# JuliaParallel/DistributedArrays.jl

Hardware: AMD Instinct MI355X
Metric: sum(DArray) GB/s (higher is better)
Workload: dtype f64; 1 GPU; cfg2: sum(drand(Float64, 2^28)) per GPU, 1-D block distribution; per_gpu_elems=268435456, global_elems=268435456

## Files before the change

distributedarrays_jl_amd/_ffi.py:

```python
import ctypes
import os

_HERE = os.path.dirname(os.path.abspath(__file__))
_SO = os.path.join(_HERE, "libdarray_hip.so")

if not os.path.exists(_SO):
    raise ImportError(
        "libdarray_hip.so is missing (%s). Build it first: "
        "`python -c \"import __graft_entry__; __graft_entry__.build()\"` "
        "or `make -C distributedarrays_jl_amd/csrc`. There is no CPU "
        "fallback: the HIP extension IS the compute path." % _SO)

try:
    ctypes.CDLL("/opt/rocm/lib/libamdhip64.so", mode=ctypes.RTLD_GLOBAL)
except OSError:
    pass

lib = ctypes.CDLL(_SO)

u64 = ctypes.c_uint64
i64 = ctypes.c_int64
i32 = ctypes.c_int
f64 = ctypes.c_double
ptr = ctypes.c_void_p
# ... 57 lines not shown
    "da_sendrecv": ([ptr, i32, ptr, i32, u64], i32),
    "da_p2p_stream": ([i32], i32),
    "da_comm_after_compute": ([], i32),
    "da_main_after_comm": ([], i32),
    "da_comm_sync": ([], i32),
    "da_bcast": ([ptr, u64, i32], i32),
    "da_barrier": ([], i32),
    "da_synchronize": ([], i32),
    "da_event_create": ([ctypes.POINTER(ptr)], i32),
    "da_event_record": ([ptr], i32),
    "da_event_elapsed": ([ptr, ptr, ctypes.POINTER(ctypes.c_float)], i32),
    "da_event_destroy": ([ptr], i32),
    "da_errstr": ([i32], ctypes.c_char_p),
    "da_device_props": ([ctypes.c_char_p, i32, ctypes.POINTER(u64)], i32),
    "da_bytes_in_use": ([], u64),
}

_dbg_sigs = {
    "dbg_reduce_dims_variant": ([u64, u64, u64], i32),
    "dbg_gemm_path": ([i64, i64, i64], i32),
}
_scan_dbg_sigs = {
    "dbg_scan_variant": ([u64, u64, u64], i32),
}
DIMS_VARIANTS = ("slices", "threads", "waves", "blocks")
GEMM_PATHS = ("naive", "mfma")
SCAN_VARIANTS = ("cols", "block", "spans")
COPY_FAMILIES = ("runs", "general")
COPY_MAXND = 6

# ... 18 lines not shown
```

distributedarrays_jl_amd/csrc/abi.hip:

```cpp
#include "common.hpp"
#include <stdarg.h>
#include <stdio.h>
#include <stdlib.h>
#include <unistd.h>
#include <errno.h>
#include <time.h>

namespace da {

static State g_state;
State& st() { return g_state; }

char g_errbuf[1024] = "ok";

int set_err(int code, const char* fmt, ...) {
    va_list ap;
    va_start(ap, fmt);
    vsnprintf(g_errbuf, sizeof(g_errbuf), fmt, ap);
    va_end(ap);
    return code;
}

int ensure_scratch(size_t bytes) {
    if (st().scratch_bytes >= bytes) return 0;
// ... 45 lines not shown
int da_init(int device, int rank, int nranks, const char* rccl_uid_path) {
    if (st().inited) return 0;
    if (nranks < 1 || rank < 0 || rank >= nranks)
        return set_err(-2, "da_init: bad rank %d/%d", rank, nranks);
    DA_CHECK_HIP(hipSetDevice(device));
    DA_CHECK_HIP(hipStreamCreateWithFlags(&st().stream, hipStreamNonBlocking));
    DA_CHECK_HIP(hipStreamCreateWithFlags(&st().comm_stream,
                                          hipStreamNonBlocking));
    DA_CHECK_HIP(hipEventCreateWithFlags(&st().ev_main,
                                         hipEventDisableTiming));
    DA_CHECK_HIP(hipEventCreateWithFlags(&st().ev_comm,
                                         hipEventDisableTiming));
    DA_CHECK_HIP(hipMalloc(&st().red_ticket, sizeof(unsigned int)));
    DA_CHECK_HIP(hipMemset(st().red_ticket, 0, sizeof(unsigned int)));
    st().red_base = 0;
    DA_CHECK_HIP(hipHostMalloc(&st().red_host, 16, hipHostMallocDefault));
    memset(st().red_host, 0, 16);
    DA_CHECK_HIP(hipHostGetDevicePointer(&st().red_host_dev,
                                         st().red_host, 0));
    st().device = device;
    st().rank = rank;
    st().nranks = nranks;
    if (nranks > 1) {
        if (!rccl_uid_path)
            return set_err(-2, "da_init: nranks>1 needs a uid path");
        ncclUniqueId uid;
        if (rank == 0) {
            DA_CHECK_NCCL(ncclGetUniqueId(&uid));
            char tmp[1024];
            snprintf(tmp, sizeof(tmp), "%s.tmp", rccl_uid_path);
            FILE* f = fopen(tmp, "wb");
            if (!f) return set_err(-4, "da_init: cannot write %s", tmp);
// ... 381 lines not shown
    return dbg_mfma_probe_impl(DA_F32, A, B, nullptr, out_raw, st().stream);
}

int dbg_reduce_dims_variant(uint64_t inner, uint64_t axis, uint64_t outer) {
    return reduce_dims_variant(inner, axis, outer);
}

int dbg_gemm_path(int64_t m, int64_t n, int64_t k) {
    return gemm_path(m, n, k);
}

int dbg_scan_variant(uint64_t inner, uint64_t axis, uint64_t outer) {
    return scan_variant(inner, axis, outer);
}


int da_group_start(void) {
    DA_REQUIRE_INIT();
    DA_CHECK_NCCL(ncclGroupStart());
    return 0;
}

int da_group_end(void) {
    DA_REQUIRE_INIT();
    DA_CHECK_NCCL(ncclGroupEnd());
    return 0;
}

static hipStream_t p2p_stream() {
    return st().p2p_comm ? st().comm_stream : st().stream;
// ... 131 lines not shown
```

distributedarrays_jl_amd/csrc/common.hpp:

```cpp
#pragma once
#include <hip/hip_runtime.h>
#include <rccl/rccl.h>
#include <stdint.h>
#include <stdio.h>
#include <string.h>
#include <mutex>
#include <unordered_map>

#include "darray_hip.h"

namespace da {

struct State {
    bool inited = false;
    int device = 0;
    int rank = 0;
    int nranks = 1;
    hipStream_t stream = nullptr;
    hipStream_t comm_stream = nullptr;
    bool p2p_comm = false;
    hipEvent_t ev_main = nullptr, ev_comm = nullptr;
    ncclComm_t comm = nullptr;
    void* scratch = nullptr;
    size_t scratch_bytes = 0;
    void* partials = nullptr;
    size_t partials_bytes = 0;
    unsigned int* red_ticket = nullptr;
    unsigned int red_base = 0;
    void* red_host = nullptr;
    void* red_host_dev = nullptr;
    std::mutex mem_mtx;
    std::unordered_map<void*, uint64_t> allocs;
    uint64_t bytes_in_use = 0;
    std::unordered_map<uint64_t, std::vector<void*>> pool;
    uint64_t pool_bytes = 0;
};

State& st();

extern char g_errbuf[1024];
int set_err(int code, const char* fmt, ...);

#define DA_CHECK_HIP(expr) do {                                          \
    hipError_t _e = (expr);                                              \
    if (_e != hipSuccess)                                                \
// ... 17 lines not shown
    switch (dtype) {
        case DA_F64: return 8;
        case DA_F32: return 4;
        case DA_I64: return 8;
    }
    return 0;
}

int ensure_scratch(size_t bytes);
int ensure_partials(size_t bytes);

constexpr int RMAXB = 8192;
int reduce_grid(uint64_t want);
bool reduce_fused_on();
int reduce_stage2_launch(int redop, int g, int dtype, hipStream_t s);
int reduce_result(void* out_host, size_t bytes, hipStream_t s);

template <typename L>
inline int fanin_launch(int g, L launch) {
    DA_CHECK_HIP(launch(st().red_base));
    st().red_base += (unsigned int)g;
    return 0;
}

int launch_fill(void* chunk, double v, uint64_t n, int dtype, hipStream_t s);
int launch_rand(void* chunk, uint64_t n, int dtype, uint64_t seed, int kind,
                uint64_t offset, hipStream_t s);
int launch_map(int opcode, void* dst, const void* src, uint64_t n, int dtype,
               hipStream_t s);
int launch_map2(int opcode, void* dst, const void* a, const void* b,
                uint64_t n, int dtype, hipStream_t s);
int launch_bcast_fma(void* d, const void* a, const void* b, double c,
                     uint64_t n, int dtype, hipStream_t s);
int launch_map2_scalar(int opcode, void* dst, const void* src, double c,
                       int rev, uint64_t n, int dtype, hipStream_t s);
int launch_expr(const int32_t* prog, int plen, void* dst,
                const uint64_t* dst_dims, int nd,
// ... 80 lines not shown
```

distributedarrays_jl_amd/csrc/embedded_src.hpp:

```cpp
#pragma once
static const char embedded_mapops_hpp[] = R"EMBED(// mapops.hpp — the unary/binary scalar functor tables shared by the
// map/map2 kernels (kernels_elementwise.hip) and the fused-broadcast
// expression interpreter (kernels_expr.hip).  ONE source of truth for
// numerics: da_expr of a single-op program is bit-identical to da_map.
//
// Semantics follow the reference's scalar-math list
// (/root/reference/test/darray.jl:775-800) with Julia conventions
// (sign/round/sinc/cosc/mod noted inline); compiled -ffp-contract=off.
#pragma once
#include "darray_hip.h"
#include "fastmath.hpp"

namespace da {

// -------------------------------------------------------------------- map
// Unary functors.  Julia-compatible semantics noted where non-obvious.
template <typename T> struct MathF;
template <> struct MathF<double> {
    static __device__ double sin_(double x) { return sin(x); }
    static __device__ double cos_(double x) { return cos(x); }
    static __device__ double tan_(double x) { return tan(x); }
    static __device__ double exp_(double x) { return exp(x); }
    static __device__ double log_(double x) { return log(x); }
    static __device__ double sqrt_(double x) { return sqrt(x); }
// ... 382 lines not shown
// ticket - base == g - 1 in unsigned arithmetic; that holds across
// wrap-around, any sequence of grid sizes, and interleaved dtypes /
// reduce / count / expression-reduce calls.
template <typename A>
__device__ __forceinline__ void publish_partial(A* p, A v) {
    if constexpr (sizeof(A) == 8)
        __hip_atomic_store((unsigned long long*)p,
                           __builtin_bit_cast(unsigned long long, v),
                           __ATOMIC_RELAXED, __HIP_MEMORY_SCOPE_AGENT);
    else
        __hip_atomic_store((unsigned int*)p,
                           __builtin_bit_cast(unsigned int, v),
                           __ATOMIC_RELAXED, __HIP_MEMORY_SCOPE_AGENT);
}

// `acc`: the block's partial (valid in thread 0).  `sh`: RTPB/64 + 1
// shared elements — block_reduce_in's scratch plus the "I am last"
// flag, kept in ONE __shared__ object.  Reusing sh[0..3] for the final
// fold is safe: wave 0 read them before it wrote the flag, and every
// other wave writes them again only after the barriers below.
template <typename A>
__device__ __forceinline__ void fanin_finish(int redop, A acc, A* partials,
                                             unsigned int* ticket,
                                             unsigned int base, A* out,
                                             A* sh) {
    if (threadIdx.x == 0) {
        publish_partial(partials + blockIdx.x, acc);
        __asm__ volatile("s_waitcnt vmcnt(0)" ::: "memory");
        unsigned int t = __hip_atomic_fetch_add(
            ticket, 1u, __ATOMIC_RELAXED, __HIP_MEMORY_SCOPE_AGENT);
        sh[RTPB / 64] = (t - base == gridDim.x - 1) ? (A)1 : (A)0;
    }
    __syncthreads();
    if (sh[RTPB / 64] == (A)0) return;
    // guide order: the fence, that lane's vmcnt wait, the barrier
    if (threadIdx.x == 0) {
        __builtin_amdgcn_fence(__ATOMIC_ACQUIRE, "agent");
        __asm__ volatile("s_waitcnt vmcnt(0)" ::: "memory");
    }
    __syncthreads();
    A facc = RedIdent<A>::get(redop);
    for (unsigned int j = threadIdx.x; j < gridDim.x; j += RTPB)
        facc = red_comb(redop, facc, partials[j]);
    facc = block_reduce_in(redop, facc, sh);
    if (threadIdx.x == 0) out[0] = facc;
}

} // namespace da
)EMBED";
static const char embedded_darray_hip_h[] = R"EMBED(/* darray_hip.h — C ABI of libdarray_hip.so: the MI355X-native local-compute
 * path for DistributedArrays.jl-style distributed arrays.
 *
 * This is the drop-in boundary of SURVEY.md §8(b): each entry point replaces
 * one worker-side local operation of the reference (citations below are
 * file:line into /root/reference).  The reference touches localparts only
 * through the init-constructor / localpart / fan-out seam
 * (src/darray.jl:76-118, :330-337; src/broadcast.jl:80; src/mapreduce.jl:31;
 * src/linalg.jl:224), so a Julia caller binds these with plain `ccall`
 * (see INTEGRATION.md) and keeps every other line of the reference.
 *
// ... 170 lines not shown
 * hipRTC (cached per process; DA_EXPR_JIT=0 forces the interpreter).
 * state: 1 ready, 2 active, -1 hipRTC failed (interpreter fallback). */
int da_expr_jit_state(void);
const char* da_expr_jit_errstr(void);
/* Fused mapreduce over a program: op-folds (da_expr_reduce) or counts the
 * nonzero terms of (da_expr_count; exact, NaN counts) the program's values
 * over a local chunk of n elements WITHOUT materialising them — one
 * launch, one read per operand element, result in *out (host; the dtype's
 * own scalar / an int64_t).  Program arguments as da_expr; dims is the
 * local chunk shape reduced over; src_strides == NULL means every operand
 * is dense over it (f64/f32/i64, any n), else the strided variant
 * (f64/f32, nd <= 4, n < 2^32).  n == 0 gives the fold identity / 0.
 * Fold-order contract: *out has EXACTLY the bits of da_expr into a dense
 * temporary followed by da_reduce(DA_REDF_IDENTITY, redop, tmp, n) /
 * da_count(DA_REDF_NONZERO, tmp, n) in the same process (DA_RV4 does not
 * apply; DA_RED_FUSED=0 and DA_EXPR_JIT=0 are honoured, same bits). */
int da_expr_reduce(const int32_t* prog, int prog_len,
                   const uint64_t* dims, int nd,
                   void* const* srcs, const uint64_t* src_strides, int nsrcs,
                   const double* consts, int nconsts, uint64_t n, int dtype,
                   int redop, void* out);
int da_expr_count(const int32_t* prog, int prog_len,
                  const uint64_t* dims, int nd,
                  void* const* srcs, const uint64_t* src_strides, int nsrcs,
                  const double* consts, int nconsts, uint64_t n, int dtype,
                  int64_t* out);
int da_map2_scalar(int opcode, void* dst, const void* src, double c,
                   int reverse, uint64_t n, int dtype);      /* D .+ 1 etc (scalar broadcast arg, broadcast.jl:124-133) */
int da_axpby(void* y, const void* x, double alpha, double beta,
             uint64_t n, int dtype);                         /* y = alpha*x + beta*y: axpy! linalg.jl:24-34 */
int da_add(void* dest, const void* src, double scale,
           uint64_t n, int dtype);                           /* add!, linalg.jl:62-76 */
int da_scale(void* a, double s, uint64_t n, int dtype);      /* rmul!, linalg.jl:54-59 */
/* dtype conversion (DArray{T2}(D) family); float->i64 rounds half-even */
int da_cast(void* dst, int dst_dtype, const void* src, int src_dtype,
            uint64_t n);

/* ---- reductions -------------------------------------------------------*/
/* Local (per-chunk) mapreduce stage: LDS + wavefront-shuffle tree.
 * Result written to *out as the dtype's own scalar type (f64/f32/i64) —
 * the per-worker mapreduce(f, op, localpart(d)) of mapreduce.jl:31.
 * n == 0 returns the fold identity. */
int da_reduce(int mapop, int redop, const void* src, uint64_t n, int dtype,
              void* out);
/* Exact predicate count (count(f, A), mapreduce.jl:115-122): mapop must be
 * a predicate (DA_REDF_ISNAN / ISFINITE / NONZERO).  The 0/1 values are
 * accumulated in a 64-bit integer on the device whatever the source dtype,
 * so *out is exact for every n (a float accumulator rounds above 2^24).
 * Fold across ranks with da_allreduce(out, 1, DA_I64, DA_RED_ADD). */
int da_count(int mapop, const void* src, uint64_t n, int dtype,
             int64_t* out);
/* Per-chunk dims-reduction (src/mapreduce.jl:42-94, mapreducedim_within):
 * chunk viewed column-major as (inner, axis, outer); dst gets
 * inner*outer elements reduced over axis (identity when axis==0). */
int da_reduce_dims(int mapop, int redop, const void* src, uint64_t inner,
                   uint64_t axis, uint64_t outer, int dtype, void* dst);
/* Inclusive scan (Base.accumulate / cumsum / cumprod) of a local chunk viewed
 * column-major as (inner, axis, outer), along `axis`:
 *   dst[i + inner*(k + axis*o)] =
 *       [carry[i + inner*o] (op)] src[i,0,o] (op) src[i,1,o] (op) .. (op) src[i,k,o]
 * redop is a da_redop (ADD, MUL, MIN, MAX; NaN-propagating min/max and
 * wrap-around i64 exactly as da_reduce), dtype f64/f32/i64, accumulation in
 * the dtype itself; the bracketing of a float sum or product is unspecified
 * (a tree over tiles and spans), like the reductions'.  carry is a device
// ... 89 lines not shown
enum da_dims_variant { DA_DIMS_SLICES = 0, DA_DIMS_THREADS, DA_DIMS_WAVES,
                       DA_DIMS_BLOCKS };
enum da_gemm_path_id { DA_GEMM_NAIVE = 0, DA_GEMM_MFMA = 1 };
/* cols: inner > 1, one thread per line; block: inner == 1, one workgroup
 * per line (>= 512 lines, or lines of at most one 2048-element tile);
 * spans: inner == 1, fewer and longer lines, cut into spans, two launches */
enum da_scan_variant { DA_SCAN_COLS = 0, DA_SCAN_BLOCK, DA_SCAN_SPANS };
/* kernel family da_reduce_dims picks for a (inner, axis, outer) view */
int dbg_reduce_dims_variant(uint64_t inner, uint64_t axis, uint64_t outer);
/* MFMA or naive kernel for da_gemm_f64/f32 at (m, n, k), k > 0, alpha != 0 */
int dbg_gemm_path(int64_t m, int64_t n, int64_t k);
/* kernel family da_scan picks for a (inner, axis, outer) view (spelled
 * `extern int`: tests/test_abi.py pins the set of plain `int dbg_*`
 * declarations to the two selectors above) */
extern int dbg_scan_variant(uint64_t inner, uint64_t axis, uint64_t outer);

/* ---- introspection / errors ------------------------------------------ */
const char* da_errstr(int code);
int da_device_props(char* name, int name_len, uint64_t* hbm_bytes);
uint64_t da_bytes_in_use(void);   /* leak check hook (test/runtests.jl:28-37 analog) */

#ifdef __cplusplus
}
#endif
#endif /* DARRAY_HIP_H */
)EMBED";
```

distributedarrays_jl_amd/csrc/expr_jit.hip:

```cpp
#include "common.hpp"
#include "embedded_src.hpp"
#include <hip/hiprtc.h>
#include <stdlib.h>
#include <string>
#include <unordered_map>
#include <vector>

namespace da {

static_assert(DA_EXPR_MAXARGS == 6 && DA_EXPR_MAXCONSTS == 6 &&
              DA_EXPR_MAXND == 4,
              "JARGS_DECL literal must be kept in sync");
struct JArgs {
    void* dst;
    const void* srcs[DA_EXPR_MAXARGS];
    double consts[DA_EXPR_MAXCONSTS];
    unsigned long long n;
    unsigned int dims[DA_EXPR_MAXND];
    unsigned int str[DA_EXPR_MAXARGS][DA_EXPR_MAXND];
};

namespace {

struct JitEntry {
// ... 183 lines not shown
            "}\n", tname, tname, nd, nd, nsrcs > 0 ? nsrcs : 1,
            nsrcs > 0 ? nsrcs : 1, nd);
        s += buf;
    }
    return s;
}

const char* JRARGS_DECL =
    "struct JRArgs {\n"
    "  JArgs a;\n"
    "  void* partials;\n"
    "  unsigned int* ticket;\n"
    "  void* out;\n"
    "  unsigned int base;\n"
    "  int fused;\n"
    "};\n";

std::string gen_reduce_source(const int32_t* prog, int plen, int dtype,
                              int nd, int nsrcs, bool strided, int redop) {
    const bool count = redop == DA_EXPR_COUNT;
    const char* tname = dtype == DA_F64 ? "double"
                        : dtype == DA_F32 ? "float" : "long long";
    const char* aname = (count || dtype == DA_I64) ? "int64_t" : tname;
    const int rop = count ? (int)DA_RED_ADD : redop;
    std::string s =
        "#ifndef M_PI\n#define M_PI 3.14159265358979323846\n#endif\n"
        "#include \"mapops.hpp\"\n#include \"reduce_core.hpp\"\n";
    s += JARGS_DECL;
    s += JRARGS_DECL;
    s += gen_eval(prog, plen, tname, dtype == DA_I64, strided);
// ... 36 lines not shown
        "  unsigned long long st = (unsigned long long)gridDim.x * "
        "da::RTPB;\n"
        "  %s acc = da::RedIdent<%s>::get(%d);\n"
        "  unsigned long long nv = a.n / 2;\n"
        "  for (unsigned long long j = i; j < nv; j += st) {\n"
        "    %s r0 = term(a, 2 * j);\n"
        "    %s r1 = term(a, 2 * j + 1);\n"
        "    acc = ABSORB(acc, r0);\n"
        "    acc = ABSORB(acc, r1);\n"
        "  }\n"
        "  for (unsigned long long j = 2 * nv + i; j < a.n; j += st)\n"
        "    acc = ABSORB(acc, term(a, j));\n"
        "  acc = da::block_reduce_in(%d, acc, sh);\n"
        "  if (r.fused)\n"
        "    da::fanin_finish(%d, acc, (%s*)r.partials, r.ticket, r.base, "
        "(%s*)r.out, sh);\n"
        "  else if (threadIdx.x == 0)\n"
        "    ((%s*)r.partials)[blockIdx.x] = acc;\n"
        "}\n",
        count ? "count" : "reduce", aname, aname, aname, rop, tname, tname,
        rop, rop, aname, aname, aname);
    s += buf;
    return s;
}

int jit_compile(const std::string& src, std::vector<char>* code) {
    const char* hdr_names[] = {"stdint.h", "darray_hip.h", "mapops.hpp",
                               "fastmath.hpp", "reduce_core.hpp"};
    const char* stdint_stub =
        "#pragma once\n"
        "typedef __INT8_TYPE__ int8_t;\ntypedef __UINT8_TYPE__ uint8_t;\n"
// ... 113 lines not shown
    uint64_t b = (work + 255) / 256;
    if (b > 8192) b = 8192;
    if (b == 0) b = 1;
    DA_CHECK_HIP(hipModuleLaunchKernel(fn, (unsigned)b, 1, 1, 256, 1, 1,
                                       0, s, nullptr, cfg));
    return 0;
}

struct JRArgs {
    JArgs a;
    void* partials;
    unsigned int* ticket;
    void* out;
    unsigned int base;
    int fused;
};

int launch_expr_reduce_jit(const int32_t* prog, int plen,
                           const uint64_t* dims, int nd, void* const* srcs,
                           const uint64_t* src_strides, int nsrcs,
                           const double* consts, int nconsts, uint64_t n,
                           int dtype, int redop, int g, bool fused,
                           hipStream_t s) {
    const char* e = getenv("DA_EXPR_JIT");
    if (e && e[0] == '0') return 1;
    if (g_jit_state < 0) return 1;
    bool strided = src_strides != nullptr;
    std::string src = gen_reduce_source(prog, plen, dtype, nd, nsrcs,
                                        strided, redop);
    hipFunction_t fn;
// ... 6 lines not shown
    JRArgs r;
    memset(&r, 0, sizeof(r));
    for (int i = 0; i < nsrcs; ++i) r.a.srcs[i] = srcs[i];
    for (int i = 0; i < nconsts; ++i) r.a.consts[i] = consts[i];
    r.a.n = n;
    if (strided) {
        for (int d = 0; d < nd; ++d) r.a.dims[d] = (unsigned)dims[d];
        for (int k = 0; k < nsrcs; ++k)
            for (int d = 0; d < nd; ++d)
                r.a.str[k][d] = (unsigned)src_strides[(size_t)k * nd + d];
    }
    r.partials = st().partials;
    r.ticket = st().red_ticket;
    r.out = st().red_host_dev;
    r.fused = fused ? 1 : 0;
    auto launch = [&](unsigned int base) {
        r.base = base;
        size_t rsz = sizeof(r);
        void* cfg[] = {HIP_LAUNCH_PARAM_BUFFER_POINTER, &r,
                       HIP_LAUNCH_PARAM_BUFFER_SIZE, &rsz,
                       HIP_LAUNCH_PARAM_END};
        return hipModuleLaunchKernel(fn, (unsigned)g, 1, 1, 256, 1, 1, 0, s,
                                     nullptr, cfg);
    };
    if (fused) return fanin_launch(g, launch);
    DA_CHECK_HIP(launch(0u));
    return 0;
}

int expr_jit_state() { return g_jit_state; }
const char* expr_jit_err() { return g_jit_err; }

}

extern "C" int dbg_expr_jit_compile(const int32_t* prog, int plen,
                                    int dtype, int nd, int nsrcs,
                                    int strided, char* src_out,
                                    int src_len) {
    using namespace da;
    std::string src = gen_source(prog, plen, dtype, nd, nsrcs,
                                 strided != 0, 1);
// ... 28 lines not shown
```

distributedarrays_jl_amd/csrc/kernels_expr.hip:

```cpp
#include "common.hpp"
#include "mapops.hpp"
#include "reduce_core.hpp"
#include <math.h>

namespace da {

namespace {
constexpr int TPB = 256;
constexpr int MAXBLOCKS = 8192;

static inline int nblocks(uint64_t work) {
    uint64_t b = (work + TPB - 1) / TPB;
    if (b > (uint64_t)MAXBLOCKS) b = MAXBLOCKS;
    if (b == 0) b = 1;
    return (int)b;
}
}

struct ExprProg {
    int32_t ins[DA_EXPR_MAXLEN];
    int len;
    const void* srcs[DA_EXPR_MAXARGS];
    double consts[DA_EXPR_MAXCONSTS];
};
// ... 245 lines not shown
                                                 uint64_t i) {
        return expr_eval_i64(p, i);
    }
};

template <bool COUNT, typename A, typename T>
__device__ __forceinline__ A expr_absorb(int redop, A acc, T x) {
    if constexpr (COUNT) return acc + (x != (T)0 ? 1 : 0);
    else return red_comb(redop, acc, x);
}

template <typename T, typename A, bool COUNT, bool STRIDED>
__global__ void expr_reduce_kernel(ExprProg p, ExprStrides s, uint64_t n,
                                   int redop, A* partials,
                                   unsigned int* ticket, unsigned int base,
                                   int fused, A* out) {
    __shared__ A sh[RTPB / 64 + 1];
    auto term = [&](uint64_t i) -> T {
        if constexpr (STRIDED) return expr_strided_eval<T>(p, s, i);
        else return ExprTerm<T>::at(p, i);
    };
    if (COUNT) redop = DA_RED_ADD;
    uint64_t i = (uint64_t)blockIdx.x * RTPB + threadIdx.x;
    uint64_t stride = (uint64_t)gridDim.x * RTPB;
    A acc = RedIdent<A>::get(redop);
    uint64_t nv = n / 2;
    for (uint64_t j = i; j < nv; j += stride) {
        T r0 = term(2 * j);
        T r1 = term(2 * j + 1);
        acc = expr_absorb<COUNT>(redop, acc, r0);
        acc = expr_absorb<COUNT>(redop, acc, r1);
    }
    for (uint64_t j = 2 * nv + i; j < n; j += stride)
        acc = expr_absorb<COUNT>(redop, acc, term(j));
    acc = block_reduce_in(redop, acc, sh);
    if (fused)
        fanin_finish(redop, acc, partials, ticket, base, out, sh);
    else if (threadIdx.x == 0)
        partials[blockIdx.x] = acc;
}

namespace {
struct ExprRedArgs {
    ExprProg P;
    ExprStrides S;
    uint64_t n;
    int redop, g;
    bool fused;
    hipStream_t s;
};

template <typename T, typename A, bool COUNT, bool STRIDED>
int expr_reduce_interp(const ExprRedArgs& a) {
    A* parts = (A*)st().partials;
    A* out = (A*)st().red_host_dev;
    auto launch = [&](unsigned int base) {
        hipLaunchKernelGGL((expr_reduce_kernel<T, A, COUNT, STRIDED>),
                           dim3(a.g), dim3(RTPB), 0, a.s, a.P, a.S, a.n,
                           a.redop, parts, st().red_ticket, base,
                           a.fused ? 1 : 0, out);
        return hipGetLastError();
    };
    if (a.fused) return fanin_launch(a.g, launch);
    DA_CHECK_HIP(launch(0u));
    return 0;
}

template <typename T, bool STRIDED>
int expr_reduce_interp_t(const ExprRedArgs& a, bool count) {
    return count ? expr_reduce_interp<T, int64_t, true, STRIDED>(a)
                 : expr_reduce_interp<T, T, false, STRIDED>(a);
}
}

int launch_expr_reduce(const int32_t* prog, int plen, const uint64_t* dims,
                       int nd, void* const* srcs,
                       const uint64_t* src_strides, int nsrcs,
                       const double* consts, int nconsts, uint64_t n,
                       int dtype, int redop, void* out_host, hipStream_t s) {
// ... 62 lines not shown
            rc = expr_reduce_interp_t<int64_t, false>(a, count);
        else if (dtype == DA_F64)
            rc = strided ? expr_reduce_interp_t<double, true>(a, count)
                         : expr_reduce_interp_t<double, false>(a, count);
        else
            rc = strided ? expr_reduce_interp_t<float, true>(a, count)
                         : expr_reduce_interp_t<float, false>(a, count);
        if (rc) return rc;
    }
    if (!fused) {
        rc = reduce_stage2_launch(count ? (int)DA_RED_ADD : redop, g,
                                  count ? (int)DA_I64 : dtype, s);
        if (rc) return rc;
    }
    return reduce_result(out_host, count ? sizeof(int64_t)
                                         : dtype_size(dtype), s);
}

}
```

distributedarrays_jl_amd/csrc/kernels_reduce.hip:

```cpp
#include "common.hpp"
#include "reduce_core.hpp"
#include <stdlib.h>

namespace da {

int reduce_grid(uint64_t want) {
    static int cap = -1;
    if (cap < 0) {
        const char* e = getenv("DA_RBLOCKS");
        cap = e ? atoi(e) : 2048;
        if (cap < 1 || cap > RMAXB) cap = 2048;
    }
    if (want < 1) want = 1;
    return (int)(want > (uint64_t)cap ? (uint64_t)cap : want);
}

static inline bool reduce_v4() {
    static int v = -1;
    if (v < 0) {
        const char* e = getenv("DA_RV4");
        v = e ? atoi(e) : 0;
    }
    return v == 1;
}
// ... 25 lines not shown
template <typename T>
__device__ __forceinline__ T block_reduce(int redop, T v) {
    __shared__ T lds[RTPB / 64];
    return block_reduce_in(redop, v, lds);
}

template <int W, typename T, typename A, typename F>
__device__ __forceinline__ A grid_accumulate(const T* __restrict__ src,
                                             uint64_t n, A acc, F fold) {
    uint64_t i = (uint64_t)blockIdx.x * RTPB + threadIdx.x;
    uint64_t stride = (uint64_t)gridDim.x * RTPB;
    using V = T __attribute__((ext_vector_type(W)));
    uint64_t nv = n / W;
    const V* sv = reinterpret_cast<const V*>(src);
    for (uint64_t j = i; j < nv; j += stride) {
        V v = sv[j];
#pragma unroll
        for (int k = 0; k < W; ++k) acc = fold(acc, (T)v[k]);
    }
    for (uint64_t j = W * nv + i; j < n; j += stride)
        acc = fold(acc, src[j]);
    return acc;
}

template <typename T, int MOP = -1, int ROP = -1>
__global__ void reduce_stage1(int mapop, int redop, const T* __restrict__ src,
                              uint64_t n, T* __restrict__ partials) {
    if (MOP >= 0) mapop = MOP;
    if (ROP >= 0) redop = ROP;
    T acc = grid_accumulate<2>(src, n, RedIdent<T>::get(redop),
        [=](T a, T x) { return red_comb(redop, a, mapf<T>(mapop, x)); });
// ... 4 lines not shown
template <typename T, int MOP = -1, int ROP = -1>
__global__ void reduce_stage1_v4(int mapop, int redop,
                                 const T* __restrict__ src, uint64_t n,
                                 T* __restrict__ partials) {
    if (MOP >= 0) mapop = MOP;
    if (ROP >= 0) redop = ROP;
    T acc = grid_accumulate<4>(src, n, RedIdent<T>::get(redop),
        [=](T a, T x) { return red_comb(redop, a, mapf<T>(mapop, x)); });
    acc = block_reduce(redop, acc);
    if (threadIdx.x == 0) partials[blockIdx.x] = acc;
}

template <typename T, int MOP = -1, int ROP = -1>
__global__ void reduce_fused(int mapop, int redop, const T* __restrict__ src,
                             uint64_t n, T* partials, unsigned int* ticket,
                             unsigned int base, T* out) {
    if (MOP >= 0) mapop = MOP;
    if (ROP >= 0) redop = ROP;
    __shared__ T sh[RTPB / 64 + 1];
    T acc = grid_accumulate<2>(src, n, RedIdent<T>::get(redop),
        [=](T a, T x) { return red_comb(redop, a, mapf<T>(mapop, x)); });
    acc = block_reduce_in(redop, acc, sh);
    fanin_finish(redop, acc, partials, ticket, base, out, sh);
}

template <typename T>
__global__ void reduce_stage2(int redop, const T* __restrict__ partials,
                              int np, T* __restrict__ out) {
    T acc = RedIdent<T>::get(redop);
    for (int j = threadIdx.x; j < np; j += blockDim.x)
        acc = red_comb(redop, acc, partials[j]);
    acc = block_reduce(redop, acc);
    if (threadIdx.x == 0) out[0] = acc;
}

bool reduce_fused_on() {
    static int v = -1;
    if (v < 0) {
// ... 3 lines not shown
    return v == 1;
}

template <typename T> struct FlatArgs {
    bool fused;
    int grid, mapop, redop;
    const T* src;
    uint64_t n;
    T *parts, *out;
    hipStream_t s;
};

template <typename T, int MOP, int ROP>
static int launch_flat(const FlatArgs<T>& a) {
    if (a.fused)
        return fanin_launch(a.grid, [&](unsigned int base) {
            hipLaunchKernelGGL((reduce_fused<T, MOP, ROP>), dim3(a.grid),
                               dim3(RTPB), 0, a.s, a.mapop, a.redop, a.src,
                               a.n, a.parts, st().red_ticket, base, a.out);
            return hipGetLastError();
        });
    hipLaunchKernelGGL((reduce_stage1<T, MOP, ROP>), dim3(a.grid),
                       dim3(RTPB), 0, a.s, a.mapop, a.redop, a.src, a.n,
                       a.parts);
    DA_CHECK_HIP(hipGetLastError());
    return 0;
}

template <typename T>
static int do_reduce(int mapop, int redop, const T* src, uint64_t n,
                     void* out_host, hipStream_t s) {
    if (n == 0) {
        *(T*)out_host = RedIdent<T>::get(redop);
        return 0;
// ... 15 lines not shown
        rc = launch_flat<T, DA_REDF_ABS2, DA_RED_ADD>(a);
    else if (mapop == DA_REDF_ABS && redop == DA_RED_ADD)
        rc = launch_flat<T, DA_REDF_ABS, DA_RED_ADD>(a);
    else if (mapop == DA_REDF_IDENTITY && redop == DA_RED_MAX)
        rc = launch_flat<T, DA_REDF_IDENTITY, DA_RED_MAX>(a);
    else if (mapop == DA_REDF_IDENTITY && redop == DA_RED_MIN)
        rc = launch_flat<T, DA_REDF_IDENTITY, DA_RED_MIN>(a);
    else
        rc = launch_flat<T, -1, -1>(a);
    if (rc) return rc;
    if (!a.fused) {
        hipLaunchKernelGGL(reduce_stage2<T>, dim3(1), dim3(RTPB), 0, s,
                           redop, a.parts, g, a.out);
        DA_CHECK_HIP(hipGetLastError());
    }
    return reduce_result(out_host, sizeof(T), s);
}

template <typename T>
__device__ __forceinline__ int64_t predf(int mapop, T x) {
    switch (mapop) {
    case DA_REDF_ISNAN: return x != x ? 1 : 0;
    case DA_REDF_ISFINITE: return isfinite((double)x) ? 1 : 0;
    }
    return x != (T)0 ? 1 : 0;
}
template <>
__device__ __forceinline__ int64_t predf<int64_t>(int mapop, int64_t x) {
    return mapf(mapop, x);
}

template <typename T>
__global__ void count_stage1(int mapop, const T* __restrict__ src,
                             uint64_t n, int64_t* __restrict__ partials) {
    int64_t acc = grid_accumulate<2>(src, n, (int64_t)0,
        [=](int64_t a, T x) { return a + predf<T>(mapop, x); });
    acc = block_reduce(DA_RED_ADD, acc);
    if (threadIdx.x == 0) partials[blockIdx.x] = acc;
}

template <typename T>
__global__ void count_fused(int mapop, const T* __restrict__ src, uint64_t n,
                            int64_t* partials, unsigned int* ticket,
                            unsigned int base, int64_t* out) {
    __shared__ int64_t sh[RTPB / 64 + 1];
    int64_t acc = grid_accumulate<2>(src, n, (int64_t)0,
        [=](int64_t a, T x) { return a + predf<T>(mapop, x); });
    acc = block_reduce_in((int)DA_RED_ADD, acc, sh);
    fanin_finish((int)DA_RED_ADD, acc, partials, ticket, base, out, sh);
}

template <typename T>
static int do_count(int mapop, const T* src, uint64_t n, int64_t* out_host,
                    hipStream_t s) {
    int g = reduce_grid((n / 2 + RTPB - 1) / RTPB);
    int rc = ensure_partials(RMAXB * sizeof(double));
    if (rc) return rc;
    int64_t* parts = (int64_t*)st().partials;
    int64_t* out = (int64_t*)st().red_host_dev;
    if (reduce_fused_on()) {
        rc = fanin_launch(g, [&](unsigned int base) {
            hipLaunchKernelGGL(count_fused<T>, dim3(g), dim3(RTPB), 0, s,
                               mapop, src, n, parts, st().red_ticket, base,
                               out);
            return hipGetLastError();
        });
        if (rc) return rc;
    } else {
        hipLaunchKernelGGL(count_stage1<T>, dim3(g), dim3(RTPB), 0, s,
                           mapop, src, n, parts);
        DA_CHECK_HIP(hipGetLastError());
        hipLaunchKernelGGL(reduce_stage2<int64_t>, dim3(1), dim3(RTPB), 0, s,
                           (int)DA_RED_ADD, parts, g, out);
        DA_CHECK_HIP(hipGetLastError());
    }
    return reduce_result(out_host, sizeof(int64_t), s);
}

int launch_count(int mapop, const void* src, uint64_t n, int dtype,
                 int64_t* out_host, hipStream_t s) {
    if (mapop < DA_REDF_ISNAN || mapop > DA_REDF_NONZERO)
        return set_err(-3, "da_count: mapop %d is not a predicate", mapop);
    if (!out_host) return set_err(-3, "da_count: null out");
    if (dtype != DA_F64 && dtype != DA_F32 && dtype != DA_I64)
        return set_err(-3, "da_count: bad dtype %d", dtype);
    if (n == 0) { *out_host = 0; return 0; }
    switch (dtype) {
    case DA_F64: return do_count<double>(mapop, (const double*)src, n,
                                         out_host, s);
    case DA_F32: return do_count<float>(mapop, (const float*)src, n,
                                        out_host, s);
// ... 223 lines not shown
        break;
    case DA_F32:
        hipLaunchKernelGGL(reduce_stage2<float>, dim3(1), dim3(RTPB), 0, s,
                           redop, (const float*)st().partials, g,
                           (float*)st().red_host_dev);
        break;
    default:
        hipLaunchKernelGGL(reduce_stage2<int64_t>, dim3(1), dim3(RTPB), 0, s,
                           redop, (const int64_t*)st().partials, g,
                           (int64_t*)st().red_host_dev);
    }
    DA_CHECK_HIP(hipGetLastError());
    return 0;
}

int reduce_result(void* out_host, size_t bytes, hipStream_t s) {
    DA_CHECK_HIP(hipStreamSynchronize(s));
    memcpy(out_host, st().red_host, bytes);
    return 0;
}

}
```

distributedarrays_jl_amd/csrc/reduce_core.hpp:

```cpp
#pragma once
#include "darray_hip.h"

namespace da {

constexpr int RTPB = 256;

template <typename T> struct RedIdent {
    static __device__ __host__ T get(int redop) {
        switch (redop) {
        case DA_RED_ADD: return (T)0;
        case DA_RED_MUL: return (T)1;
        case DA_RED_MIN: return (T)__builtin_inff();
        case DA_RED_MAX: return (T)(-__builtin_inff());
        }
        return (T)0;
    }
};
template <> struct RedIdent<int64_t> {
    static __device__ __host__ int64_t get(int redop) {
        switch (redop) {
        case DA_RED_ADD: return 0;
        case DA_RED_MUL: return 1;
        case DA_RED_MIN: return __INT64_MAX__;
        case DA_RED_MAX: return -__INT64_MAX__ - 1;
// ... 44 lines not shown
}

template <typename A>
__device__ __forceinline__ void publish_partial(A* p, A v) {
    if constexpr (sizeof(A) == 8)
        __hip_atomic_store((unsigned long long*)p,
                           __builtin_bit_cast(unsigned long long, v),
                           __ATOMIC_RELAXED, __HIP_MEMORY_SCOPE_AGENT);
    else
        __hip_atomic_store((unsigned int*)p,
                           __builtin_bit_cast(unsigned int, v),
                           __ATOMIC_RELAXED, __HIP_MEMORY_SCOPE_AGENT);
}

template <typename A>
__device__ __forceinline__ void fanin_finish(int redop, A acc, A* partials,
                                             unsigned int* ticket,
                                             unsigned int base, A* out,
                                             A* sh) {
    if (threadIdx.x == 0) {
        publish_partial(partials + blockIdx.x, acc);
        __asm__ volatile("s_waitcnt vmcnt(0)" ::: "memory");
        unsigned int t = __hip_atomic_fetch_add(
            ticket, 1u, __ATOMIC_RELAXED, __HIP_MEMORY_SCOPE_AGENT);
        sh[RTPB / 64] = (t - base == gridDim.x - 1) ? (A)1 : (A)0;
    }
    __syncthreads();
    if (sh[RTPB / 64] == (A)0) return;
    if (threadIdx.x == 0) {
        __builtin_amdgcn_fence(__ATOMIC_ACQUIRE, "agent");
        __asm__ volatile("s_waitcnt vmcnt(0)" ::: "memory");
    }
    __syncthreads();
    A facc = RedIdent<A>::get(redop);
    for (unsigned int j = threadIdx.x; j < gridDim.x; j += RTPB)
        facc = red_comb(redop, facc, partials[j]);
    facc = block_reduce_in(redop, facc, sh);
    if (threadIdx.x == 0) out[0] = facc;
}

}
```

include/darray_hip.h:

```cpp
#ifndef DARRAY_HIP_H
#define DARRAY_HIP_H

#include <stdint.h>

#ifdef __cplusplus
extern "C" {
#endif

enum da_dtype { DA_F64 = 0, DA_F32 = 1, DA_I64 = 2 };

enum da_mapop {
    DA_OP_IDENTITY = 0, DA_OP_NEG, DA_OP_ABS, DA_OP_ABS2, DA_OP_INV,
    DA_OP_SQRT, DA_OP_CBRT, DA_OP_EXP, DA_OP_EXP2, DA_OP_EXP10,
    DA_OP_EXPM1, DA_OP_LOG, DA_OP_LOG2, DA_OP_LOG10, DA_OP_LOG1P,
    DA_OP_SIN, DA_OP_COS, DA_OP_TAN, DA_OP_ASIN, DA_OP_ACOS, DA_OP_ATAN,
    DA_OP_SINH, DA_OP_COSH, DA_OP_TANH, DA_OP_ASINH, DA_OP_ACOSH,
    DA_OP_ATANH, DA_OP_SINPI, DA_OP_COSPI, DA_OP_FLOOR, DA_OP_CEIL,
    DA_OP_ROUND, DA_OP_TRUNC, DA_OP_SIGN, DA_OP_DEG2RAD, DA_OP_RAD2DEG,
    DA_OP_SEC, DA_OP_CSC, DA_OP_COT,
    DA_OP_ERF, DA_OP_ERFC, DA_OP_ERFINV, DA_OP_ERFCINV, DA_OP_ERFCX,
    DA_OP_GAMMA, DA_OP_LGAMMA, DA_OP_SINC, DA_OP_COSC,
    DA_OP_SIND, DA_OP_COSD, DA_OP_TAND, DA_OP_ASIND, DA_OP_ACOSD,
    DA_OP_ATAND, DA_OP_ACOT, DA_OP_ACOTD, DA_OP_ASEC, DA_OP_ACSC,
    DA_OP_ASECH, DA_OP_ACSCH, DA_OP_ACOTH,
// ... 132 lines not shown
int da_barrier(void);

int da_synchronize(void);
int da_event_create(void** ev);
int da_event_record(void* ev);
int da_event_elapsed(void* ev_start, void* ev_stop, float* ms);
int da_event_destroy(void* ev);

enum da_dims_variant { DA_DIMS_SLICES = 0, DA_DIMS_THREADS, DA_DIMS_WAVES,
                       DA_DIMS_BLOCKS };
enum da_gemm_path_id { DA_GEMM_NAIVE = 0, DA_GEMM_MFMA = 1 };
enum da_scan_variant { DA_SCAN_COLS = 0, DA_SCAN_BLOCK, DA_SCAN_SPANS };
int dbg_reduce_dims_variant(uint64_t inner, uint64_t axis, uint64_t outer);
int dbg_gemm_path(int64_t m, int64_t n, int64_t k);
extern int dbg_scan_variant(uint64_t inner, uint64_t axis, uint64_t outer);

const char* da_errstr(int code);
int da_device_props(char* name, int name_len, uint64_t* hbm_bytes);
uint64_t da_bytes_in_use(void);

#ifdef __cplusplus
}
#endif
#endif
```

Before: 6139 GB/s.

## Poll a pinned host result slot instead of synchronising the stream after reductions

The fused single-launch reduce kernels now publish {value, sequence} into a coherent mapped pinned host slot with a system-scope release store. The host spins on that sequence word for up to DA_RED_SPIN_US microseconds before falling back to hipStreamSynchronize, which removes the stream-sync latency from each scalar reduce. The grid-accumulate loop also switches to nontemporal loads of the source. In exchange the host burns CPU while spinning, the stream is no longer guaranteed drained on return, and the slot becomes fine-grained coherent memory.

Measured after the change: 6829 GB/s, median of 6. 1.11x the previous value.

```diff
diff --git a/distributedarrays_jl_amd/_ffi.py b/distributedarrays_jl_amd/_ffi.py
--- a/distributedarrays_jl_amd/_ffi.py
+++ b/distributedarrays_jl_amd/_ffi.py
@@ -95,6 +95,7 @@
     "da_errstr": ([i32], ctypes.c_char_p),
     "da_device_props": ([ctypes.c_char_p, i32, ctypes.POINTER(u64)], i32),
     "da_bytes_in_use": ([], u64),
+    "da_dbg_reduce_waits": ([ctypes.POINTER(u64), ctypes.POINTER(u64)], i32),
 }
 
 _dbg_sigs = {
diff --git a/distributedarrays_jl_amd/csrc/abi.hip b/distributedarrays_jl_amd/csrc/abi.hip
--- a/distributedarrays_jl_amd/csrc/abi.hip
+++ b/distributedarrays_jl_amd/csrc/abi.hip
@@ -83,8 +83,11 @@
     DA_CHECK_HIP(hipMalloc(&st().red_ticket, sizeof(unsigned int)));
     DA_CHECK_HIP(hipMemset(st().red_ticket, 0, sizeof(unsigned int)));
     st().red_base = 0;
-    DA_CHECK_HIP(hipHostMalloc(&st().red_host, 16, hipHostMallocDefault));
+    DA_CHECK_HIP(hipHostMalloc(&st().red_host, 16,
+                               hipHostMallocCoherent | hipHostMallocMapped));
     memset(st().red_host, 0, 16);
+    st().red_seq = 0;
+    reduce_waits_reset();
     DA_CHECK_HIP(hipHostGetDevicePointer(&st().red_host_dev,
                                          st().red_host, 0));
     st().device = device;
@@ -496,6 +499,11 @@
     return scan_variant(inner, axis, outer);
 }
 
+int da_dbg_reduce_waits(uint64_t* polled, uint64_t* synced) {
+    reduce_waits(polled, synced);
+    return 0;
+}
+
 
 int da_group_start(void) {
     DA_REQUIRE_INIT();
diff --git a/distributedarrays_jl_amd/csrc/common.hpp b/distributedarrays_jl_amd/csrc/common.hpp
--- a/distributedarrays_jl_amd/csrc/common.hpp
+++ b/distributedarrays_jl_amd/csrc/common.hpp
@@ -29,6 +29,7 @@
     unsigned int red_base = 0;
     void* red_host = nullptr;
     void* red_host_dev = nullptr;
+    uint64_t red_seq = 0;
     std::mutex mem_mtx;
     std::unordered_map<void*, uint64_t> allocs;
     uint64_t bytes_in_use = 0;
@@ -76,13 +77,28 @@
 int reduce_grid(uint64_t want);
 bool reduce_fused_on();
 int reduce_stage2_launch(int redop, int g, int dtype, hipStream_t s);
-int reduce_result(void* out_host, size_t bytes, hipStream_t s);
+int reduce_result(void* out_host, size_t bytes, hipStream_t s, uint64_t seq);
+void reduce_waits(uint64_t* polled, uint64_t* synced);
+void reduce_waits_reset();
 
 template <typename L>
 inline int fanin_launch(int g, L launch) {
     DA_CHECK_HIP(launch(st().red_base));
     st().red_base += (unsigned int)g;
     return 0;
+}
+
+template <typename L>
+inline int fanin_launch_seq(int g, L launch) {
+    const uint64_t seq = st().red_seq + 1;
+    int rc = fanin_launch(g, [&](unsigned int base) {
+        return launch(base, (unsigned long long)seq);
+    });
+    if (rc == 0) st().red_seq = seq;
+    return rc;
+}
+inline uint64_t published_seq(bool fused) {
+    return fused ? st().red_seq : 0;
 }
 
 int launch_fill(void* chunk, double v, uint64_t n, int dtype, hipStream_t s);
diff --git a/distributedarrays_jl_amd/csrc/embedded_src.hpp b/distributedarrays_jl_amd/csrc/embedded_src.hpp
--- a/distributedarrays_jl_amd/csrc/embedded_src.hpp
+++ b/distributedarrays_jl_amd/csrc/embedded_src.hpp
@@ -420,6 +420,31 @@
                            __ATOMIC_RELAXED, __HIP_MEMORY_SCOPE_AGENT);
 }
 
+// The result hand-off to the host.  `out` is the device address of the
+// 16-byte pinned host slot { 8-byte value, 64-bit sequence } (RedSlot,
+// reduce_wait.hpp).  One lane, once per launch: a system-scope store of
+// the value, then a system-scope RELEASE store of this launch's `seq`
+// into out + 8, so a host whose acquire load of the sequence word
+// returns `seq` reads this launch's value.  The release stays a release:
+// the guide's fence-free write-through form (§6 Guideline 16 R1) is
+// stated for agent-scope hand-offs inside a launch, not for host-visible
+// memory at system scope.  Two stores, never one 16-byte one: nothing
+// promises that arrives untorn.
+template <typename A>
+__device__ __forceinline__ void publish_result(A* out, A v,
+                                               unsigned long long seq) {
+    if constexpr (sizeof(A) == 8)
+        __hip_atomic_store((unsigned long long*)out,
+                           __builtin_bit_cast(unsigned long long, v),
+                           __ATOMIC_RELAXED, __HIP_MEMORY_SCOPE_SYSTEM);
+    else
+        __hip_atomic_store((unsigned int*)out,
+                           __builtin_bit_cast(unsigned int, v),
+                           __ATOMIC_RELAXED, __HIP_MEMORY_SCOPE_SYSTEM);
+    __hip_atomic_store((unsigned long long*)((char*)out + 8), seq,
+                       __ATOMIC_RELEASE, __HIP_MEMORY_SCOPE_SYSTEM);
+}
+
 // `acc`: the block's partial (valid in thread 0).  `sh`: RTPB/64 + 1
 // shared elements — block_reduce_in's scratch plus the "I am last"
 // flag, kept in ONE __shared__ object.  Reusing sh[0..3] for the final
@@ -429,6 +454,7 @@
 __device__ __forceinline__ void fanin_finish(int redop, A acc, A* partials,
                                              unsigned int* ticket,
                                              unsigned int base, A* out,
+                                             unsigned long long seq,
                                              A* sh) {
     if (threadIdx.x == 0) {
         publish_partial(partials + blockIdx.x, acc);
@@ -449,7 +475,7 @@
     for (unsigned int j = threadIdx.x; j < gridDim.x; j += RTPB)
         facc = red_comb(redop, facc, partials[j]);
     facc = block_reduce_in(redop, facc, sh);
-    if (threadIdx.x == 0) out[0] = facc;
+    if (threadIdx.x == 0) publish_result(out, facc, seq);
 }
 
 } // namespace da
@@ -650,7 +676,9 @@
  * Fold-order contract: *out has EXACTLY the bits of da_expr into a dense
  * temporary followed by da_reduce(DA_REDF_IDENTITY, redop, tmp, n) /
  * da_count(DA_REDF_NONZERO, tmp, n) in the same process (DA_RV4 does not
- * apply; DA_RED_FUSED=0 and DA_EXPR_JIT=0 are honoured, same bits). */
+ * apply; DA_RED_FUSED=0 and DA_EXPR_JIT=0 are honoured, same bits).
+ * Like da_reduce, neither call drains the stream (stream contract under
+ * "reductions" below). */
 int da_expr_reduce(const int32_t* prog, int prog_len,
                    const uint64_t* dims, int nd,
                    void* const* srcs, const uint64_t* src_strides, int nsrcs,
@@ -673,17 +701,31 @@
             uint64_t n);
 
 /* ---- reductions -------------------------------------------------------*/
+/* Stream contract of the scalar results (da_reduce, da_count,
+ * da_expr_reduce, da_expr_count): the call returns once *out holds the
+ * result, and by then the reducing kernel has finished READING its
+ * sources.  It does NOT promise that the rank's stream has drained: the
+ * single-launch kernel publishes {value, sequence} into a pinned host slot
+ * and the host watches that slot for up to DA_RED_SPIN_US microseconds
+ * (default 2000) instead of synchronising the stream.  Work queued before
+ * the reduce has completed (one stream, in order); the runtime may not yet
+ * know.  A caller that needs the stream drained (to read other device
+ * results through its own channel, say) calls da_synchronize.  The stream
+ * is synchronised as before when the budget runs out (a kernel fault comes
+ * back as the HIP error then), with DA_RED_SPIN_US=0, and on the
+ * two-kernel path (DA_RED_FUSED=0, DA_RV4=1). */
 /* Local (per-chunk) mapreduce stage: LDS + wavefront-shuffle tree.
  * Result written to *out as the dtype's own scalar type (f64/f32/i64) —
  * the per-worker mapreduce(f, op, localpart(d)) of mapreduce.jl:31.
- * n == 0 returns the fold identity. */
+ * n == 0 returns the fold identity.  Does not drain the stream (above). */
 int da_reduce(int mapop, int redop, const void* src, uint64_t n, int dtype,
               void* out);
 /* Exact predicate count (count(f, A), mapreduce.jl:115-122): mapop must be
  * a predicate (DA_REDF_ISNAN / ISFINITE / NONZERO).  The 0/1 values are
  * accumulated in a 64-bit integer on the device whatever the source dtype,
  * so *out is exact for every n (a float accumulator rounds above 2^24).
- * Fold across ranks with da_allreduce(out, 1, DA_I64, DA_RED_ADD). */
+ * Fold across ranks with da_allreduce(out, 1, DA_I64, DA_RED_ADD).
+ * Does not drain the stream (stream contract above). */
 int da_count(int mapop, const void* src, uint64_t n, int dtype,
              int64_t* out);
 /* Per-chunk dims-reduction (src/mapreduce.jl:42-94, mapreducedim_within):
@@ -803,6 +845,10 @@
  * `extern int`: tests/test_abi.py pins the set of plain `int dbg_*`
  * declarations to the two selectors above) */
 extern int dbg_scan_variant(uint64_t inner, uint64_t axis, uint64_t outer);
+/* how many scalar results (da_reduce, da_count, da_expr_reduce,
+ * da_expr_count) were taken from the poll of the pinned slot and how many
+ * from the stream-sync fallback since da_init; either pointer may be NULL */
+int da_dbg_reduce_waits(uint64_t* polled, uint64_t* synced);
 
 /* ---- introspection / errors ------------------------------------------ */
 const char* da_errstr(int code);
diff --git a/distributedarrays_jl_amd/csrc/expr_jit.hip b/distributedarrays_jl_amd/csrc/expr_jit.hip
--- a/distributedarrays_jl_amd/csrc/expr_jit.hip
+++ b/distributedarrays_jl_amd/csrc/expr_jit.hip
@@ -221,6 +221,7 @@
     "  void* out;\n"
     "  unsigned int base;\n"
     "  int fused;\n"
+    "  unsigned long long seq;\n"
     "};\n";
 
 std::string gen_reduce_source(const int32_t* prog, int plen, int dtype,
@@ -287,7 +288,7 @@
         "  acc = da::block_reduce_in(%d, acc, sh);\n"
         "  if (r.fused)\n"
         "    da::fanin_finish(%d, acc, (%s*)r.partials, r.ticket, r.base, "
-        "(%s*)r.out, sh);\n"
+        "(%s*)r.out, r.seq, sh);\n"
         "  else if (threadIdx.x == 0)\n"
         "    ((%s*)r.partials)[blockIdx.x] = acc;\n"
         "}\n",
@@ -431,6 +432,7 @@
     void* out;
     unsigned int base;
     int fused;
+    unsigned long long seq;
 };
 
 int launch_expr_reduce_jit(const int32_t* prog, int plen,
@@ -467,8 +469,9 @@
     r.ticket = st().red_ticket;
     r.out = st().red_host_dev;
     r.fused = fused ? 1 : 0;
-    auto launch = [&](unsigned int base) {
+    auto launch = [&](unsigned int base, unsigned long long seq) {
         r.base = base;
+        r.seq = seq;
         size_t rsz = sizeof(r);
         void* cfg[] = {HIP_LAUNCH_PARAM_BUFFER_POINTER, &r,
                        HIP_LAUNCH_PARAM_BUFFER_SIZE, &rsz,
@@ -476,8 +479,8 @@
         return hipModuleLaunchKernel(fn, (unsigned)g, 1, 1, 256, 1, 1, 0, s,
                                      nullptr, cfg);
     };
-    if (fused) return fanin_launch(g, launch);
-    DA_CHECK_HIP(launch(0u));
+    if (fused) return fanin_launch_seq(g, launch);
+    DA_CHECK_HIP(launch(0u, 0ull));
     return 0;
 }
 
diff --git a/distributedarrays_jl_amd/csrc/kernels_expr.hip b/distributedarrays_jl_amd/csrc/kernels_expr.hip
--- a/distributedarrays_jl_amd/csrc/kernels_expr.hip
+++ b/distributedarrays_jl_amd/csrc/kernels_expr.hip
@@ -283,7 +283,8 @@
 __global__ void expr_reduce_kernel(ExprProg p, ExprStrides s, uint64_t n,
                                    int redop, A* partials,
                                    unsigned int* ticket, unsigned int base,
-                                   int fused, A* out) {
+                                   int fused, A* out,
+                                   unsigned long long seq) {
     __shared__ A sh[RTPB / 64 + 1];
     auto term = [&](uint64_t i) -> T {
         if constexpr (STRIDED) return expr_strided_eval<T>(p, s, i);
@@ -304,7 +305,7 @@
         acc = expr_absorb<COUNT>(redop, acc, term(j));
     acc = block_reduce_in(redop, acc, sh);
     if (fused)
-        fanin_finish(redop, acc, partials, ticket, base, out, sh);
+        fanin_finish(redop, acc, partials, ticket, base, out, seq, sh);
     else if (threadIdx.x == 0)
         partials[blockIdx.x] = acc;
 }
@@ -323,15 +324,15 @@
 int expr_reduce_interp(const ExprRedArgs& a) {
     A* parts = (A*)st().partials;
     A* out = (A*)st().red_host_dev;
-    auto launch = [&](unsigned int base) {
+    auto launch = [&](unsigned int base, unsigned long long seq) {
         hipLaunchKernelGGL((expr_reduce_kernel<T, A, COUNT, STRIDED>),
                            dim3(a.g), dim3(RTPB), 0, a.s, a.P, a.S, a.n,
                            a.redop, parts, st().red_ticket, base,
-                           a.fused ? 1 : 0, out);
+                           a.fused ? 1 : 0, out, seq);
         return hipGetLastError();
     };
-    if (a.fused) return fanin_launch(a.g, launch);
-    DA_CHECK_HIP(launch(0u));
+    if (a.fused) return fanin_launch_seq(a.g, launch);
+    DA_CHECK_HIP(launch(0u, 0ull));
     return 0;
 }
 
@@ -424,7 +425,8 @@
         if (rc) return rc;
     }
     return reduce_result(out_host, count ? sizeof(int64_t)
-                                         : dtype_size(dtype), s);
-}
-
-}
+                                         : dtype_size(dtype), s,
+                         published_seq(fused));
+}
+
+}
diff --git a/distributedarrays_jl_amd/csrc/kernels_reduce.hip b/distributedarrays_jl_amd/csrc/kernels_reduce.hip
--- a/distributedarrays_jl_amd/csrc/kernels_reduce.hip
+++ b/distributedarrays_jl_amd/csrc/kernels_reduce.hip
@@ -1,5 +1,6 @@
 #include "common.hpp"
 #include "reduce_core.hpp"
+#include "reduce_wait.hpp"
 #include <stdlib.h>
 
 namespace da {
@@ -63,7 +64,7 @@
     uint64_t nv = n / W;
     const V* sv = reinterpret_cast<const V*>(src);
     for (uint64_t j = i; j < nv; j += stride) {
-        V v = sv[j];
+        V v = __builtin_nontemporal_load(&sv[j]);
 #pragma unroll
         for (int k = 0; k < W; ++k) acc = fold(acc, (T)v[k]);
     }
@@ -98,14 +99,15 @@
 template <typename T, int MOP = -1, int ROP = -1>
 __global__ void reduce_fused(int mapop, int redop, const T* __restrict__ src,
                              uint64_t n, T* partials, unsigned int* ticket,
-                             unsigned int base, T* out) {
+                             unsigned int base, T* out,
+                             unsigned long long seq) {
     if (MOP >= 0) mapop = MOP;
     if (ROP >= 0) redop = ROP;
     __shared__ T sh[RTPB / 64 + 1];
     T acc = grid_accumulate<2>(src, n, RedIdent<T>::get(redop),
         [=](T a, T x) { return red_comb(redop, a, mapf<T>(mapop, x)); });
     acc = block_reduce_in(redop, acc, sh);
-    fanin_finish(redop, acc, partials, ticket, base, out, sh);
+    fanin_finish(redop, acc, partials, ticket, base, out, seq, sh);
 }
 
 template <typename T>
@@ -139,10 +141,12 @@
 template <typename T, int MOP, int ROP>
 static int launch_flat(const FlatArgs<T>& a) {
     if (a.fused)
-        return fanin_launch(a.grid, [&](unsigned int base) {
+        return fanin_launch_seq(a.grid, [&](unsigned int base,
+                                            unsigned long long seq) {
             hipLaunchKernelGGL((reduce_fused<T, MOP, ROP>), dim3(a.grid),
                                dim3(RTPB), 0, a.s, a.mapop, a.redop, a.src,
-                               a.n, a.parts, st().red_ticket, base, a.out);
+                               a.n, a.parts, st().red_ticket, base, a.out,
+                               seq);
             return hipGetLastError();
         });
     hipLaunchKernelGGL((reduce_stage1<T, MOP, ROP>), dim3(a.grid),
@@ -188,7 +192,7 @@
                            redop, a.parts, g, a.out);
         DA_CHECK_HIP(hipGetLastError());
     }
-    return reduce_result(out_host, sizeof(T), s);
+    return reduce_result(out_host, sizeof(T), s, published_seq(a.fused));
 }
 
 template <typename T>
@@ -216,12 +220,14 @@
 template <typename T>
 __global__ void count_fused(int mapop, const T* __restrict__ src, uint64_t n,
                             int64_t* partials, unsigned int* ticket,
-                            unsigned int base, int64_t* out) {
+                            unsigned int base, int64_t* out,
+                            unsigned long long seq) {
     __shared__ int64_t sh[RTPB / 64 + 1];
     int64_t acc = grid_accumulate<2>(src, n, (int64_t)0,
         [=](int64_t a, T x) { return a + predf<T>(mapop, x); });
     acc = block_reduce_in((int)DA_RED_ADD, acc, sh);
-    fanin_finish((int)DA_RED_ADD, acc, partials, ticket, base, out, sh);
+    fanin_finish((int)DA_RED_ADD, acc, partials, ticket, base, out, seq,
+                 sh);
 }
 
 template <typename T>
@@ -233,10 +239,11 @@
     int64_t* parts = (int64_t*)st().partials;
     int64_t* out = (int64_t*)st().red_host_dev;
     if (reduce_fused_on()) {
-        rc = fanin_launch(g, [&](unsigned int base) {
+        rc = fanin_launch_seq(g, [&](unsigned int base,
+                                     unsigned long long seq) {
             hipLaunchKernelGGL(count_fused<T>, dim3(g), dim3(RTPB), 0, s,
                                mapop, src, n, parts, st().red_ticket, base,
-                               out);
+                               out, seq);
             return hipGetLastError();
         });
         if (rc) return rc;
@@ -248,7 +255,8 @@
                            (int)DA_RED_ADD, parts, g, out);
         DA_CHECK_HIP(hipGetLastError());
     }
-    return reduce_result(out_host, sizeof(int64_t), s);
+    return reduce_result(out_host, sizeof(int64_t), s,
+                         published_seq(reduce_fused_on()));
 }
 
 int launch_count(int mapop, const void* src, uint64_t n, int dtype,
@@ -502,9 +510,41 @@
     return 0;
 }
 
-int reduce_result(void* out_host, size_t bytes, hipStream_t s) {
+static uint64_t red_spin_us() {
+    static int64_t v = -1;
+    if (v < 0) {
+        const char* e = getenv("DA_RED_SPIN_US");
+        v = e ? atoll(e) : 2000;
+        if (v < 0) v = 2000;
+    }
+    return (uint64_t)v;
+}
+
+static uint64_t g_red_polled = 0, g_red_synced = 0;
+
+void reduce_waits(uint64_t* polled, uint64_t* synced) {
+    if (polled) *polled = g_red_polled;
+    if (synced) *synced = g_red_synced;
+}
+void reduce_waits_reset() { g_red_polled = g_red_synced = 0; }
+
+int reduce_result(void* out_host, size_t bytes, hipStream_t s,
+                  uint64_t seq) {
+    const RedSlot* slot = (const RedSlot*)st().red_host;
+    const uint64_t budget = seq ? red_spin_us() : 0;
+    if (budget && red_wait(slot, seq, budget, out_host, bytes)) {
+        ++g_red_polled;
+        return 0;
+    }
     DA_CHECK_HIP(hipStreamSynchronize(s));
-    memcpy(out_host, st().red_host, bytes);
+    if (seq && __atomic_load_n(&slot->seq, __ATOMIC_ACQUIRE) != seq)
+        return set_err(-6, "flat reduce: the stream drained but the result "
+                       "slot holds sequence %llu, not %llu",
+                       (unsigned long long)__atomic_load_n(
+                           &slot->seq, __ATOMIC_RELAXED),
+                       (unsigned long long)seq);
+    memcpy(out_host, slot->value, bytes);
+    ++g_red_synced;
     return 0;
 }
 
diff --git a/distributedarrays_jl_amd/csrc/reduce_core.hpp b/distributedarrays_jl_amd/csrc/reduce_core.hpp
--- a/distributedarrays_jl_amd/csrc/reduce_core.hpp
+++ b/distributedarrays_jl_amd/csrc/reduce_core.hpp
@@ -82,9 +82,25 @@
 }
 
 template <typename A>
+__device__ __forceinline__ void publish_result(A* out, A v,
+                                               unsigned long long seq) {
+    if constexpr (sizeof(A) == 8)
+        __hip_atomic_store((unsigned long long*)out,
+                           __builtin_bit_cast(unsigned long long, v),
+                           __ATOMIC_RELAXED, __HIP_MEMORY_SCOPE_SYSTEM);
+    else
+        __hip_atomic_store((unsigned int*)out,
+                           __builtin_bit_cast(unsigned int, v),
+                           __ATOMIC_RELAXED, __HIP_MEMORY_SCOPE_SYSTEM);
+    __hip_atomic_store((unsigned long long*)((char*)out + 8), seq,
+                       __ATOMIC_RELEASE, __HIP_MEMORY_SCOPE_SYSTEM);
+}
+
+template <typename A>
 __device__ __forceinline__ void fanin_finish(int redop, A acc, A* partials,
                                              unsigned int* ticket,
                                              unsigned int base, A* out,
+                                             unsigned long long seq,
                                              A* sh) {
     if (threadIdx.x == 0) {
         publish_partial(partials + blockIdx.x, acc);
@@ -104,7 +120,7 @@
     for (unsigned int j = threadIdx.x; j < gridDim.x; j += RTPB)
         facc = red_comb(redop, facc, partials[j]);
     facc = block_reduce_in(redop, facc, sh);
-    if (threadIdx.x == 0) out[0] = facc;
+    if (threadIdx.x == 0) publish_result(out, facc, seq);
 }
 
 }
diff --git a/distributedarrays_jl_amd/csrc/reduce_wait.hpp b/distributedarrays_jl_amd/csrc/reduce_wait.hpp
--- /dev/null
+++ b/distributedarrays_jl_amd/csrc/reduce_wait.hpp
@@ -0,0 +1,41 @@
+#pragma once
+#include <stdint.h>
+#include <string.h>
+#include <chrono>
+
+namespace da {
+
+struct RedSlot {
+    unsigned char value[8];
+    uint64_t seq;
+};
+static_assert(sizeof(RedSlot) == 16, "pinned result slot is 16 bytes");
+
+inline void cpu_pause() {
+#if defined(__x86_64__) || defined(__i386__)
+    __builtin_ia32_pause();
+#elif defined(__aarch64__)
+    __asm__ volatile("yield");
+#endif
+}
+
+constexpr unsigned RED_POLLS_PER_CLOCK = 256;
+
+inline bool red_wait(const RedSlot* slot, uint64_t seq, uint64_t budget_us,
+                     void* out, size_t bytes) {
+    using clock = std::chrono::steady_clock;
+    const clock::time_point deadline =
+        clock::now() + std::chrono::microseconds(budget_us);
+    for (;;) {
+        for (unsigned k = 0; k < RED_POLLS_PER_CLOCK; ++k) {
+            if (__atomic_load_n(&slot->seq, __ATOMIC_ACQUIRE) == seq) {
+                memcpy(out, slot->value, bytes);
+                return true;
+            }
+            cpu_pause();
+        }
+        if (clock::now() >= deadline) return false;
+    }
+}
+
+}
diff --git a/include/darray_hip.h b/include/darray_hip.h
--- a/include/darray_hip.h
+++ b/include/darray_hip.h
@@ -170,6 +170,7 @@
 int dbg_reduce_dims_variant(uint64_t inner, uint64_t axis, uint64_t outer);
 int dbg_gemm_path(int64_t m, int64_t n, int64_t k);
 extern int dbg_scan_variant(uint64_t inner, uint64_t axis, uint64_t outer);
+int da_dbg_reduce_waits(uint64_t* polled, uint64_t* synced);
 
 const char* da_errstr(int code);
 int da_device_props(char* name, int name_len, uint64_t* hbm_bytes);
```
